# HamidGadirov/OpticalFlowSciVis

Measured on AMD Instinct MI355X. Metric: volume-pairs/sec, Flow-3D unsupervised train step (fwd+loss+bwd+AdamW), higher is better.
Workload: dtype f32

## Files before the change

include/flowsci_hip.h:

```cpp
#ifndef FLOWSCI_HIP_H
#define FLOWSCI_HIP_H

#ifdef __cplusplus
extern "C" {
#endif

typedef void* fs_stream_t;

enum {
  FS_OK = 0,
  FS_ERR_NULLPTR = 1,
  FS_ERR_SHAPE = 2,
  FS_ERR_ARG = 3,
  FS_ERR_LAUNCH = 4,
  FS_ERR_UNSUPPORTED = 5
};

#define FS_ABI_VERSION 330
int fs_version(void);
const char* fs_error_string(int code);

int fs_warp3d_fwd(const float* in, const float* flow, float* out,
                  int B, int C, const int* in_dhw, int D, int H, int W, fs_stream_t stream);
int fs_warp3d_bwd(const float* in, const float* flow, const float* grad_out,
// ... 188 lines not shown
long long fs_conv3d_fwd_dprelu_part_floats(int B, int Cout, int Do, int Ho, int Wo);
long long fs_conv3d_fwd_dprelu_part_floats_k3(int B, int Cout, int Do, int Ho, int Wo);
int fs_conv3d_fwd_dprelu(const float* x, const float* w, const float* act_y, const float* prelu_weight,
                         int num_prelu_weights, float* grad_act_y, float* grad_prelu_weight, float* grad_bias,
                         float* part, float* ws, int B, int Cin, int Cout, int Di, int Hi, int Wi, int Do, int Ho, int Wo,
                         int kernel, int stride, int pad, fs_stream_t stream);
int fs_conv3d_fwd_prelu(const float* x, const float* w, const float* bias, const float* prelu_weight,
                        const float* residual, float* y, float* z, float* ws,
                        int B, int Cin, int Cout, int Di, int Hi, int Wi, int Do, int Ho, int Wo,
                        int kernel, int stride, int pad, int num_prelu_weights, fs_stream_t stream);
int fs_conv3d_tr_prelu(const float* x, const float* w, const float* bias, const float* prelu_weight,
                       float* y, float* z, float* ws,
                       int B, int Cin, int Cout, int Di, int Hi, int Wi, int Dout, int Hout, int Wout,
                       int num_prelu_weights, fs_stream_t stream);
int fs_conv3d_tr_add(const float* x, const float* w, const float* bias, const float* addend, float* y,
                     float* ws, int B, int Cin, int Cout, int Di, int Hi, int Wi,
                     int Dout, int Hout, int Wout, fs_stream_t stream);
long long fs_conv3d_tr_ws_floats(int Cin, int Cout);
int fs_conv3d_tr(const float* x, const float* w, const float* bias, float* y, float* ws,
                 int B, int Cin, int Cout, int Di, int Hi, int Wi, int Dout, int Hout, int Wout,
                 fs_stream_t stream);

#define FS_PRELU_MAX_CHUNKS 64
int fs_prelu_bwd(const float* x, const float* grad_out, const float* weight,
                 float* grad_x, float* grad_weight, float* grad_bias, float* ws,
                 int B, int C, int S, int num_weights, fs_stream_t stream);

int fs_conv3d_wrw(const float* g, const float* src, float* dw, int B, int Cg, int Cs,
                  int Do, int Ho, int Wo, int Di, int Hi, int Wi,
                  int kernel, int stride, int pad, fs_stream_t stream);
enum { FS_WRW_KERNEL_BRICK = 0,
       FS_WRW_KERNEL_DMA = 1,
       FS_WRW_KERNEL_WINO23 = 2,
       FS_WRW_KERNEL_WINO43 = 3    };
int fs_conv3d_wrw_kernel_id(const float* g, const float* src, int B, int Cg, int Cs,
                            int Do, int Ho, int Wo, int Di, int Hi, int Wi, int kernel, int stride, int pad);

int fs_conv3d_fwd_prelu_ms(const float* const* src, const long long* batch_strides, const float* w, const float* bias,
                           const float* prelu_weight, float* y, float* z, float* ws,
                           int B, int Cin, int Cout, int Di, int Hi, int Wi, int Do, int Ho, int Wo,
                           int kernel, int stride, int pad, int num_prelu_weights, fs_stream_t stream);
int fs_conv3d_wrw_ms(const float* g, const float* const* src, const long long* batch_strides, float* dw,
                     int B, int Cg, int Cs, int Do, int Ho, int Wo, int Di, int Hi, int Wi,
                     int kernel, int stride, int pad, fs_stream_t stream);

long long fs_conv3d_wrw_det_ws_floats(const float* g, const float* src, const float* const* src_planes,
                                      const long long* batch_strides, int B, int Cg, int Cs,
                                      int Do, int Ho, int Wo, int Di, int Hi, int Wi, int kernel, int stride, int pad);
int fs_conv3d_wrw_det(const float* g, const float* src, const float* const* src_planes, const long long* batch_strides,
                      float* dw, float* ws, long long ws_floats, int B, int Cg, int Cs,
                      int Do, int Ho, int Wo, int Di, int Hi, int Wi, int kernel, int stride, int pad,
                      fs_stream_t stream);

typedef struct FsWprepJob {
  const float* w;
  float* ws;
  int kind;
  int total;
  int p[6];
} FsWprepJob;
int fs_conv3d_fwd_wprep_jobs(FsWprepJob* jobs_host, int cap, const float* x, const float* w, float* ws,
                             int B, int Cin, int Cout, int Di, int Hi, int Wi, int Do, int Ho, int Wo,
                             int kernel, int stride, int pad, int wmode);
int fs_conv3d_tr_wprep_jobs(FsWprepJob* jobs_host, int cap, const float* x, const float* w, float* ws, int B, int Cin,
                            int Cout, int Di, int Hi, int Wi, int Dout, int Hout, int Wout, int has_prelu_out);
int fs_conv3d_wprep_batch(const FsWprepJob* jobs_dev, int njobs, fs_stream_t stream);

// ... 5 lines not shown
```

opticalflowscivis_amd/csrc/convwrw.hip:

```cpp
#include <cstdint>
#include <cstdlib>
#include <type_traits>

#include "common.hpp"

namespace {

typedef float f32x16 __attribute__((ext_vector_type(16)));

constexpr int KW = 32;

struct WP {
  int B, Cg, Cs;
  int Do, Ho, Wo;
  int Di, Hi, Wi;
  int pad;
  int segs;
  long long steps;
  int spw;
  int nsrc = 0;
  const float* const* srcv = nullptr;
  const long long* sbsv = nullptr;
};

struct WB {
  int B, Cg, Cs;
  int Do, Ho, Wo, Di, Hi, Wi;
  int pad;
  int bz, by, bx;
  long long bricks;
  int spw;
  int nsrc;
  const float* src[12];
  long long sbs[12];
  long long slab;
};

struct WDet {
  float* ws;
  long long cap;
  long long* need;
};

__global__ __launch_bounds__(256) void wrw_reduce_kernel(const float* __restrict__ ws, int runs, long long n,
                                                         float* __restrict__ dW) {
  for (long long i = (long long)blockIdx.x * 256 + threadIdx.x; i < n; i += (long long)gridDim.x * 256) {
    float a = ws[i];
    for (int r = 1; r < runs; ++r) a += ws[(size_t)r * n + i];
    dW[i] = a;
  }
}

static inline int wrw_det_begin(const WDet* det, long long runs, long long dwf, float* dW, float** out, long long* p_slab) {
  *out = dW; *p_slab = 0;
  if (det == nullptr) return -1;
  if (det->need != nullptr) { *det->need = runs * dwf; return FS_OK; }
  if (det->ws == nullptr || runs * dwf > det->cap) return FS_ERR_ARG;
  *out = det->ws; *p_slab = dwf;
  return -1;
}

static inline void wrw_det_end(const WDet* det, long long runs, long long dwf, float* dW, hipStream_t st) {
  if (det == nullptr || det->need != nullptr) return;
  const long long blocks = (dwf + 255) / 256;
  hipLaunchKernelGGL(wrw_reduce_kernel, dim3((unsigned)(blocks < 4096 ? blocks : 4096)), dim3(256), 0, st, det->ws, (int)runs,
                     dwf, dW);
}

// ... 204 lines not shown
  if (want < 1) want = 1;
  long long spw = (p.bricks + want - 1) / want;
  if (spw < 2) spw = 2;
  p.spw = (int)(spw > (1 << 20) ? (1 << 20) : spw);
  const long long gx = (p.bricks + p.spw - 1) / p.spw;
  if (gx >= (1ll << 31) || nchunks > 65535 || mtiles > 65535) return FS_ERR_SHAPE;
  dim3 grid((unsigned)gx, nchunks, mtiles);
  constexpr int K3 = K * K * K;
  float* out;
  const long long dwf = (long long)p.Cg * p.Cs * K3;
  const int drc = wrw_det_begin(det, gx, dwf, dW, &out, &p.slab);
  if (drc >= 0) return drc;
  if (mt == 2)
    hipLaunchKernelGGL((conv3d_wrw_brick_kernel<K, S, NC, 2, TZ, TY>), grid, dim3(256), 0, st, G, Src, out, p);
  else
    hipLaunchKernelGGL((conv3d_wrw_brick_kernel<K, S, NC, 1, TZ, TY>), grid, dim3(256), 0, st, G, Src, out, p);
  wrw_det_end(det, gx, dwf, dW, st);
  FS_LAUNCH_CHECK();
  return FS_OK;
}


typedef __attribute__((address_space(3))) void* lds_ptr_t;
constexpr unsigned DMA_OOB = 0x80000000u;
#ifdef FS_WRW_STAMPS
__device__ unsigned long long fs_wrw_dbg[4 * 8];
#define STAMP(i) do { const unsigned long long now_ = __builtin_amdgcn_s_memtime(); dt[i] += now_ - tprev; tprev = now_; } while (0)
#else
#define STAMP(i) do { } while (0)
#endif

constexpr int up4(int n) { return (n + 3) / 4 * 4; }

template <int K, int S, int NC, int MT, int TZ, int TY, int FULL, int HALF, int KWX = 32>
__global__ __launch_bounds__(512, 2) void conv3d_wrw_dma_kernel(const float* __restrict__ G,
                                                             const float* __restrict__ Src,
                                                             float* __restrict__ dW, WB p) {
  constexpr int K3 = K * K * K;
  constexpr int NTOT = NC * K3;
  constexpr int NT32 = 4 * FULL + 2 * HALF;
  static_assert(NT32 * 32 >= NTOT && (NT32 - 1) * 32 < NTOT + 32, "column tiles cover the chunk");
  static_assert(HALF == 0 || MT == 2, "a shared column tile is split by row tile");
  constexpr int NB = FULL + HALF;
  constexpr int ROWS = TZ * TY;
  static_assert(KWX == 32 || KWX == 16, "brick x extent");
  constexpr int YR = KW / KWX;
  constexpr int TYB = TY * YR;
  constexpr int ZT = (TZ - 1) * S + K, YT = (TYB - 1) * S + K;
  constexpr int XL = 4;
  constexpr int XP = up4(XL + (KWX - 1) * S + K);
  constexpr int PSP = YT * XP, CHSP = ZT * PSP;
  constexpr int GP = ROWS * KW + 4;
  constexpr int NGF = 32 * MT * GP;
  constexpr int NGL = (NGF + 255) / 256 * 256;
  constexpr int NSF = NC * CHSP;
  constexpr int NSL = (NSF + 255) / 256 * 256;
  constexpr int NGW = (NGL / 256 + 3) / 4;
  constexpr int NSW = (NSL / 256 + 3) / 4;
  constexpr int BUF = NGL + NSL;
  static_assert(2 * BUF * 4 <= 160 * 1024, "two buffers fit the CU's LDS");
  __shared__ __attribute__((aligned(16))) float lds[2 * BUF];

  const int t = threadIdx.x, lane = t & 63;
  const int wave = __builtin_amdgcn_readfirstlane(t >> 6);
  const int wv = wave & 3;
  const bool loader = wave >= 4;
  const int l31 = lane & 31, kh = lane >> 5;
  const int c0 = blockIdx.y * NC;
  const int g0 = blockIdx.z * 32 * MT;
  const size_t gvol = (size_t)p.Do * p.Ho * p.Wo, svol = (size_t)p.Di * p.Hi * p.Wi;
  const long long s0 = (long long)blockIdx.x * p.spw;
  const long long s1 = min(s0 + p.spw, p.bricks);

  if (loader) {
#if defined(__HIP_DEVICE_COMPILE__)
    __builtin_amdgcn_s_setprio(3);
    unsigned soff[NSW], scls[NSW];
    int sch[NSW];
    const int zhi = p.Di + p.pad - (p.bz - 1) * TZ * S, yhi = p.Hi + p.pad - (p.by - 1) * TYB * S,
              xhi = p.Wi + XL - (p.bx - 1) * KWX * S;
#pragma unroll
    for (int k = 0; k < NSW; ++k) {
      const int q = 256 * (wv + 4 * k) + 4 * lane;
      const int c = q / CHSP, r1 = q - c * CHSP;
      const int z = r1 / PSP, r2 = r1 - z * PSP;
      const int y = r2 / XP, x = r2 - y * XP;
      const bool ok = q < NSF && c0 + c < p.Cs;
      soff[k] = ok ? ((p.nsrc ? 0u : (unsigned)c * (unsigned)svol) + ((unsigned)z * p.Hi + (unsigned)y) * p.Wi + (unsigned)x) * 4u
                   : DMA_OOB;
      sch[k] = q < NSF ? c : NC - 1;
      scls[k] = (z < p.pad ? 1u : 0u) | (z >= zhi ? 2u : 0u) | (y < p.pad ? 4u : 0u) | (y >= yhi ? 8u : 0u) |
                (x < XL ? 16u : 0u) | (x >= xhi ? 32u : 0u);
    }
    unsigned goff[NGW], gpk[NGW];
#pragma unroll
    for (int k = 0; k < NGW; ++k) {
      const int f = 256 * (wv + 4 * k) + 4 * lane;
      const int r = f / GP, w = f - r * GP;
      const int row = w / KW, e = w % KW;
      const int rz = row / TY, ry = (row % TY) * YR + e / KWX, col = e % KWX;
      const bool ok = f < NGF && w < ROWS * KW && g0 + r < p.Cg;
      goff[k] = ok ? ((unsigned)r * (unsigned)gvol + (unsigned)((rz * p.Ho + ry) * p.Wo + col)) * 4u : DMA_OOB;
      gpk[k] = (unsigned)rz | ((unsigned)ry << 8) | ((unsigned)col << 16);
    }
    const bool g_exact = p.Do % TZ == 0 && p.Ho % TYB == 0 && p.Wo % KWX == 0;
    int bxi, byi, bzi, b;
    {
// ... 38 lines not shown
        __amdgpu_buffer_rsrc_t rc[NC];
#pragma unroll
        for (int c = 0; c < NC; ++c) {
          const bool live = c0 + c < p.Cs;
          const int ch = live ? c0 + c : 0;
          rc[c] = __builtin_amdgcn_make_buffer_rsrc((void*)(p.src[ch] + (size_t)b * (size_t)p.sbs[ch] + org), (short)0,
                                                    live ? 0x7fffffff : 0, 0x00020000);
        }
#pragma unroll
        for (int k = 0; k < NSW; ++k) {
          if (256 * (wv + 4 * k) < NSL) {
            const unsigned vo = (scls[k] & bmask) == 0u ? soff[k] : DMA_OOB;
#pragma unroll
            for (int c = 0; c < NC; ++c)
              if (256 * (wv + 4 * k) < (c + 1) * CHSP && 256 * (wv + 4 * k) + 256 > c * CHSP)
                if (sch[k] == c)
                  __builtin_amdgcn_raw_ptr_buffer_load_lds(rc[c], (lds_ptr_t)(dbase + NGL + 256 * (wv + 4 * k)), 16, vo, 0, 0, 0);
          }
        }
      }
      if (++bxi == p.bx) { bxi = 0; if (++byi == p.by) { byi = 0; if (++bzi == p.bz) { bzi = 0; ++b; } } }
    };
    if (s0 < s1) stage(0);
    asm volatile("s_waitcnt vmcnt(0)" ::: "memory");
    __builtin_amdgcn_s_barrier();
    int buf = 0;
    for (long long st = s0; st < s1; ++st) {
      if (st + 1 < s1) stage(buf ^ 1);
      asm volatile("s_waitcnt vmcnt(0)" ::: "memory");
      __builtin_amdgcn_s_barrier();
      buf ^= 1;
    }
#else
    (void)gvol; (void)svol; (void)NGW; (void)NSW; (void)DMA_OOB;
#endif
    return;
  }

  int boff[NB];
#pragma unroll
  for (int n = 0; n < NB; ++n) {
    const int tile = (n < FULL) ? wv * FULL + n : 4 * FULL + (wv >> 1);
    const int j = tile * 32 + l31;
    int off = 0;
    if (j < NTOT) {
      const int c = j / K3, r = j - c * K3;
      const int kz = r / (K * K), ky = (r / K) % K, kx = r % K;
      off = c * CHSP + kz * PSP + ky * XP + kx;
    }
    boff[n] = off + XL - p.pad;
  }

  f32x16 acc[FULL > 0 ? FULL : 1][MT];
  f32x16 acch;
#pragma unroll
  for (int r = 0; r < 16; ++r) {
    acch[r] = 0.f;
#pragma unroll
    for (int n = 0; n < FULL; ++n)
#pragma unroll
      for (int m = 0; m < MT; ++m) acc[n][m][r] = 0.f;
  }

  __builtin_amdgcn_s_barrier();
  int buf = 0;
#ifdef FS_WRW_STAMPS
  unsigned long long dt[8] = {0, 0, 0, 0, 0, 0, 0, 0};
  unsigned long long tprev = __builtin_amdgcn_s_memtime();
// ... 65 lines not shown

template <int K, int S, int NC, int MT, int TZ, int TY, int FULL, int HALF, int KWX = 32>
int launch_dma(const float* G, const float* Src, float* dW, const WP& w, hipStream_t st, const WDet* det = nullptr) {
  WB p;
  p.B = w.B; p.Cg = w.Cg; p.Cs = w.Cs; p.Do = w.Do; p.Ho = w.Ho; p.Wo = w.Wo;
  p.Di = w.Di; p.Hi = w.Hi; p.Wi = w.Wi; p.pad = w.pad;
  p.nsrc = w.nsrc;
  for (int c = 0; c < w.nsrc; ++c) { p.src[c] = w.srcv[c]; p.sbs[c] = w.sbsv[c]; }
  p.bz = fs::cdiv(p.Do, TZ); p.by = fs::cdiv(p.Ho, TY * (KW / KWX)); p.bx = fs::cdiv(p.Wo, KWX);
  p.bricks = (long long)p.B * p.bz * p.by * p.bx;
  const int mtiles = fs::cdiv(p.Cg, 32 * MT);
  const int nchunks = fs::cdiv(p.Cs, NC);
  long long want = 256 / ((long long)mtiles * nchunks);
  if (want < 1) want = 1;
  long long spw = (p.bricks + want - 1) / want;
  if (spw < 1) spw = 1;
  p.spw = (int)(spw > (1 << 20) ? (1 << 20) : spw);
  const long long gx = (p.bricks + p.spw - 1) / p.spw;
  if (gx >= (1ll << 31) || nchunks > 65535 || mtiles > 65535) return FS_ERR_SHAPE;
  constexpr int K3 = K * K * K;
  float* out;
  const long long dwf = (long long)p.Cg * p.Cs * K3;
  const int drc = wrw_det_begin(det, gx, dwf, dW, &out, &p.slab);
  if (drc >= 0) return drc;
  hipLaunchKernelGGL((conv3d_wrw_dma_kernel<K, S, NC, MT, TZ, TY, FULL, HALF, KWX>), dim3((unsigned)gx, nchunks, mtiles),
                     dim3(512), 0, st, G, Src, out, p);
  wrw_det_end(det, gx, dwf, dW, st);
  FS_LAUNCH_CHECK();
  return FS_OK;
}

#include "convwrwwino.hpp"
#include "convwrwwino4.hpp"

}

#ifdef FS_WRW_STAMPS
extern "C" int fs_debug_wrw_stamps(unsigned long long* out) {
  return hipMemcpyFromSymbol(out, HIP_SYMBOL(fs_wrw_dbg), sizeof(unsigned long long) * 32) == hipSuccess ? 0 : 1;
}
#endif

#define FS_WRW_PICK(id, ...)        \
  do {                              \
    if (plan != nullptr) { *plan = (id); return FS_OK; } \
    return __VA_ARGS__;             \
  } while (0)

static int conv3d_wrw_impl(const float* g, const float* src, const float* const* srcv, const long long* sbsv, float* dw,
                           int B, int Cg, int Cs, int Do, int Ho, int Wo, int Di, int Hi, int Wi, int kernel, int stride,
                           int pad, fs_stream_t stream, int* plan = nullptr, const WDet* det = nullptr) {
  FS_REQUIRE_PTR(g);
  if (plan == nullptr) FS_REQUIRE_PTR(dw);
  if (srcv == nullptr) FS_REQUIRE_PTR(src);
  if (B < 1 || Cg < 1 || Cs < 1 || Do < 1 || Ho < 1 || Wo < 1 || Di < 1 || Hi < 1 || Wi < 1)
    return FS_ERR_SHAPE;
  if (!((kernel == 3 && stride == 1) || (kernel == 4 && stride == 2)) || pad < 0 || pad >= kernel)
    return FS_ERR_ARG;
  if ((Do - 1) * stride + kernel > Di + 2 * pad || (Ho - 1) * stride + kernel > Hi + 2 * pad ||
      (Wo - 1) * stride + kernel > Wi + 2 * pad)
    return FS_ERR_SHAPE;
  if ((long long)64 * Do * Ho * Wo * 4 >= (1ll << 32) || (long long)8 * Di * Hi * Wi * 4 >= (1ll << 32))
    return FS_ERR_SHAPE;
  WP p;
  p.B = B; p.Cg = Cg; p.Cs = Cs; p.Do = Do; p.Ho = Ho; p.Wo = Wo; p.Di = Di; p.Hi = Hi; p.Wi = Wi;
  p.pad = pad;
  p.segs = fs::cdiv(Wo, KW);
  p.steps = (long long)B * Do * Ho * p.segs;
  bool ms_aligned = true;
  if (srcv != nullptr) {
    if (Cs > 12) return FS_ERR_UNSUPPORTED;
    p.nsrc = Cs; p.srcv = srcv; p.sbsv = sbsv;
    for (int c = 0; c < Cs; ++c) {
      if (srcv[c] == nullptr) return FS_ERR_NULLPTR;
      if (sbsv[c] < (long long)Di * Hi * Wi) return FS_ERR_ARG;
      ms_aligned = ms_aligned && ((uintptr_t)srcv[c] & 15) == 0 && sbsv[c] % 4 == 0;
    }
  }
  hipStream_t st = (hipStream_t)stream;
  static const bool reg_only = FS_AB_ENV("FLOWSCI_WRW_REG");
  const bool dma_ok = !reg_only && pad <= stride && (Wo >= KW || Wo == 16) && Wo % 4 == 0 && Wi % 4 == 0 &&
                      (((uintptr_t)g | (srcv ? (uintptr_t)0 : (uintptr_t)src)) & 15) == 0 && ms_aligned &&
                      (long long)64 * Do * Ho * Wo * 4 < (1ll << 31) && (long long)16 * Di * Hi * Wi * 4 < (1ll << 31);
  if (srcv != nullptr) {
    if (dma_ok && kernel == 4 && Cg <= 32 && Cs >= 3 && Wo >= KW) FS_WRW_PICK(FS_WRW_KERNEL_DMA, launch_dma<4, 2, 6, 1, 2, 2, 3, 0>(g, src, dw, p, st, det));
    return FS_ERR_UNSUPPORTED;
  }
  if (dma_ok && wrw_wino4_ok(p, g, src, kernel, stride)) FS_WRW_PICK(FS_WRW_KERNEL_WINO43, launch_wrw_wino4(g, src, dw, p, st, det));
#ifdef FS_ABLATION
  if (dma_ok && det == nullptr && wrw_wino_ok(p, g, src, kernel, stride)) FS_WRW_PICK(FS_WRW_KERNEL_WINO23, launch_wrw_wino(g, src, dw, p, st));
#endif
  if (dma_ok) {
    if (kernel == 3 && Cg > 32 && Cs >= 8 && Wo == 16) FS_WRW_PICK(FS_WRW_KERNEL_DMA, launch_dma<3, 1, 16, 2, 1, 4, 3, 1, 16>(g, src, dw, p, st, det));
    if (kernel == 3 && Cg > 32 && Cs >= 8) FS_WRW_PICK(FS_WRW_KERNEL_DMA, launch_dma<3, 1, 16, 2, 1, 4, 3, 1>(g, src, dw, p, st, det));
    if (kernel == 4 && Cg > 32 && Cs >= 4 && Wo == 16) FS_WRW_PICK(FS_WRW_KERNEL_DMA, launch_dma<4, 2, 8, 2, 1, 2, 4, 0, 16>(g, src, dw, p, st, det));
    if (kernel == 4 && Cg > 32 && Cs >= 4 && Wo >= KW) FS_WRW_PICK(FS_WRW_KERNEL_DMA, launch_dma<4, 2, 8, 2, 1, 2, 4, 0>(g, src, dw, p, st, det));
    if (kernel == 4 && Cg <= 32 && Cs >= 3 && Wo >= KW) FS_WRW_PICK(FS_WRW_KERNEL_DMA, launch_dma<4, 2, 6, 1, 2, 2, 3, 0>(g, src, dw, p, st, det));
    if (kernel == 4 && Cg <= 32 && Wo >= KW) FS_WRW_PICK(FS_WRW_KERNEL_DMA, launch_dma<4, 2, 2, 1, 2, 2, 1, 0>(g, src, dw, p, st, det));
  }
  if (kernel == 3) FS_WRW_PICK(FS_WRW_KERNEL_BRICK, launch_brick<3, 1, 8, 1, 4>(g, src, dw, p, st, det));
  const int cost2 = (Cs + 1) / 2, cost4 = 2 * ((Cs + 3) / 4);
  if (cost2 < cost4) FS_WRW_PICK(FS_WRW_KERNEL_BRICK, launch_brick<4, 2, 2, 1, 2>(g, src, dw, p, st, det));
  FS_WRW_PICK(FS_WRW_KERNEL_BRICK, launch_brick<4, 2, 4, 1, 2>(g, src, dw, p, st, det));
}

extern "C" int fs_conv3d_wrw_kernel_id(const float* g, const float* src, int B, int Cg, int Cs, int Do, int Ho, int Wo,
                                       int Di, int Hi, int Wi, int kernel, int stride, int pad) {
  int id = -1;
  const int rc = conv3d_wrw_impl(g, src, nullptr, nullptr, nullptr, B, Cg, Cs, Do, Ho, Wo, Di, Hi, Wi, kernel, stride, pad,
                                 nullptr, &id);
  return rc == FS_OK ? id : -rc;
}

extern "C" int fs_conv3d_wrw(const float* g, const float* src, float* dw, int B, int Cg, int Cs, int Do,
                             int Ho, int Wo, int Di, int Hi, int Wi, int kernel, int stride, int pad,
                             fs_stream_t stream) {
  FS_ENTER();
  return conv3d_wrw_impl(g, src, nullptr, nullptr, dw, B, Cg, Cs, Do, Ho, Wo, Di, Hi, Wi, kernel, stride, pad, stream);
}

extern "C" long long fs_conv3d_wrw_det_ws_floats(const float* g, const float* src, const float* const* src_planes,
                                                 const long long* batch_strides, int B, int Cg, int Cs, int Do, int Ho,
                                                 int Wo, int Di, int Hi, int Wi, int kernel, int stride, int pad) {
  long long need = 0;
  WDet det = {nullptr, 0, &need};
  float dummy;
  const int rc = conv3d_wrw_impl(g, src, src_planes, batch_strides, &dummy, B, Cg, Cs, Do, Ho, Wo, Di, Hi, Wi, kernel, stride,
// ... 24 lines not shown
```

opticalflowscivis_amd/ops.py:

```python
import ctypes

import torch

from . import _lib

WARP2D_RIFE, WARP2D_PWC, WARP2D_PHOTO, WARP2D_DILATED = 0, 1, 2, 3


def _stream(t):
    return torch.cuda.current_stream(t.device).cuda_stream


def _need_cuda_f32(name, t, ndim):
    if not isinstance(t, torch.Tensor):
        raise ValueError("%s must be a tensor" % name)
    if t.dtype != torch.float32:
        raise ValueError("%s must be float32, got %s" % (name, t.dtype))
    if t.dim() != ndim:
        raise ValueError("%s must be %d-D, got shape %s" % (name, ndim, tuple(t.shape)))
    if not t.is_cuda:
        raise ValueError("%s must live on a GPU (the HIP hot path has no CPU fallback); got %s" %
                         (name, t.device))
    return t.contiguous()

# ... 1499 lines not shown
    return 4 * _vol(in_dhw) * 4 < (1 << 32) and 8 * _vol(in_dhw) < (1 << 31)


def conv3d_wrw_fits(src_dhw, g_dhw):
    return 8 * _vol(src_dhw) * 4 < (1 << 32) and 64 * _vol(g_dhw) * 4 < (1 << 32)


_dw_arena = {}
_dw_need = {}


def _dw_zeros(like, shape):
    n = 1
    for v in shape:
        n *= int(v)
    if _prep_depth == 0 or not _PREP_ON or torch.cuda.is_current_stream_capturing():
        return like.new_zeros(shape)
    dev = like.device
    st = _dw_arena.get(dev)
    if st is None or st[0] != _prep_epoch:
        if st is not None:
            _dw_need[dev] = st[3]
        need = _dw_need.get(dev, 0)
        st = _dw_arena[dev] = [_prep_epoch, like.new_zeros(need) if need else None, 0, 0]
    pad = (n + 3) // 4 * 4
    st[3] += pad
    if st[1] is None or st[2] + pad > st[1].numel():
        return like.new_zeros(shape)
    out = st[1].narrow(0, st[2], n).view(shape)
    st[2] += pad
    return out


def _conv3d_wrw_det(g, src_ptr, pv, sv, geo, nbytes, flops, equiv, allow_unsupported=False):
    L = _lib.lib()
    need = int(L.fs_conv3d_wrw_det_ws_floats(g.data_ptr(), src_ptr, pv, sv, *geo))
    if need == -FS_ERR_UNSUPPORTED and allow_unsupported:
        return None
    if need < 0:
        _lib.check(-need, "fs_conv3d_wrw_det_ws_floats")
    B, Cg, Cs = geo[:3]
    k = geo[9]
    dw = g.new_empty(Cg, Cs, k, k, k)
    ws = g.new_empty(max(need, 1))
    with torch.cuda.device(g.device):
        _call("fs_conv3d_wrw_det", g.data_ptr(), src_ptr, pv, sv, dw.data_ptr(), ws.data_ptr(), need, *geo, _stream(g),
              algo_bytes=nbytes, algo_flops=flops, equiv_flops=equiv, record_as="fs_conv3d_wrw")
    return dw


def conv3d_wrw(g, src, k, stride, pad):
    g = _need_cuda_f32("g", g, 5)
    src = _need_cuda_f32("src", src, 5)
    B, Cg = g.shape[:2]
    Cs = src.shape[1]
    if src.shape[0] != B:
        raise ValueError("batch mismatch")
    fq = 2 * g.numel() * Cs * int(k) ** 3
    kid = conv3d_wrw_kernel_id(g.data_ptr(), src.data_ptr(), B, Cg, Cs, g.shape[2:], src.shape[2:], k, stride, pad)
    geo = (B, Cg, Cs, g.shape[2], g.shape[3], g.shape[4], src.shape[2], src.shape[3], src.shape[4], int(k), int(stride), int(pad))
    if torch.are_deterministic_algorithms_enabled():
        return _conv3d_wrw_det(g, src.data_ptr(), None, None, geo, 4 * (g.numel() + src.numel()),
                               {WRW_KERNEL_WINO43: fq // 2, WRW_KERNEL_WINO23: fq * 2 // 3}.get(kid, fq), fq)
    dw = _dw_zeros(g, (Cg, Cs, k, k, k))
    with torch.cuda.device(g.device):
        _call("fs_conv3d_wrw", g.data_ptr(), src.data_ptr(), dw.data_ptr(), B, Cg, Cs, g.shape[2],
              g.shape[3], g.shape[4], src.shape[2], src.shape[3], src.shape[4], int(k), int(stride),
              int(pad), _stream(g), algo_bytes=4 * (g.numel() + src.numel()),
              algo_flops={WRW_KERNEL_WINO43: fq // 2, WRW_KERNEL_WINO23: fq * 2 // 3}.get(kid, fq), equiv_flops=fq,
              kernel="conv3d_wrw_wino4_kernel<0>" if kid == WRW_KERNEL_WINO43 else None)
    return dw


WRW_KERNEL_BRICK, WRW_KERNEL_DMA, WRW_KERNEL_WINO23, WRW_KERNEL_WINO43 = 0, 1, 2, 3


def conv3d_wrw_kernel_id(g_ptr, src_ptr, B, Cg, Cs, g_dhw, src_dhw, k, stride, pad):
    kid = int(_lib.lib().fs_conv3d_wrw_kernel_id(int(g_ptr), int(src_ptr), int(B), int(Cg), int(Cs),
                                                 *(int(v) for v in g_dhw), *(int(v) for v in src_dhw), int(k), int(stride),
                                                 int(pad)))
    if kid < 0:
        _lib.check(-kid, "fs_conv3d_wrw_kernel_id")
    return kid


def conv3d_wrw_takes_winograd(B, Cg, Cs, g_dhw, src_dhw, k, stride, pad, g_misalign=0, src_misalign=0):
    return conv3d_wrw_kernel_id(0x1000 + g_misalign, 0x1000 + src_misalign, B, Cg, Cs, g_dhw, src_dhw, k, stride,
                                pad) in (WRW_KERNEL_WINO23, WRW_KERNEL_WINO43)


FS_ERR_UNSUPPORTED = 5


def _channel_planes(pieces):
    B, dhw = pieces[0].shape[0], tuple(pieces[0].shape[2:])
    vol = dhw[0] * dhw[1] * dhw[2]
    inner = (vol, dhw[1] * dhw[2], dhw[2], 1)
    ptrs, strides = [], []
    for t in pieces:
        if (not isinstance(t, torch.Tensor) or not t.is_cuda or t.dtype != torch.float32 or t.dim() != 5 or
                t.shape[0] != B or tuple(t.shape[2:]) != dhw or tuple(t.stride()[1:]) != inner or
                t.stride(0) < t.shape[1] * vol or t.stride(0) % 4 or t.data_ptr() % 16 or vol % 4):
            return None
        for c in range(t.shape[1]):
            ptrs.append(t.data_ptr() + 4 * c * vol)
            strides.append(t.stride(0))
    n = len(ptrs)
# ... 13 lines not shown
    if w.shape[1] != Cin or tuple(w.shape[2:]) != (k, k, k):
        raise ValueError("weight %s does not fit %d input channels" % (tuple(w.shape), Cin))
    if bias is not None:
        bias = _need_cuda_f32("bias", bias, 1)
    x0 = pieces[0]
    B = x0.shape[0]
    Di, Hi, Wi = x0.shape[2:]
    Do, Ho, Wo = [(n + 2 * pad - k) // stride + 1 for n in (Di, Hi, Wi)]
    if min(Do, Ho, Wo) < 1:
        return None
    y = x0.new_empty((B, Cout, Do, Ho, Wo))
    z = torch.empty_like(y)
    wp, ws = _prepared_fwd(w, x0.data_ptr(), B, Cin, Cout, (Di, Hi, Wi), (Do, Ho, Wo), k, stride, pad, 0)
    xbytes = 4 * B * Cin * Di * Hi * Wi
    with torch.cuda.device(x0.device):
        rc = _call_rc("fs_conv3d_fwd_prelu_ms", pv, sv, wp, _ptr(bias), a.data_ptr(), y.data_ptr(), z.data_ptr(),
                   ws.data_ptr(), B, Cin, Cout, Di, Hi, Wi, Do, Ho, Wo, int(k), int(stride), int(pad), int(a.numel()),
                      _stream(x0), algo_bytes=xbytes + 8 * y.numel(), algo_flops=2 * y.numel() * Cin * int(k) ** 3,
                      record_as="fs_conv3d_fwd", allow=(FS_ERR_UNSUPPORTED,))
    if rc == FS_ERR_UNSUPPORTED:
        _prep_not_written()
        return None
    return y, z


def conv3d_wrw_ms(g, pieces, k, stride, pad):
    planes = _channel_planes(pieces)
    if planes is None:
        return None
    pv, sv, Cs = planes
    g = _need_cuda_f32("g", g, 5)
    B, Cg = g.shape[:2]
    Di, Hi, Wi = pieces[0].shape[2:]
    if torch.are_deterministic_algorithms_enabled():
        geo = (B, Cg, Cs, g.shape[2], g.shape[3], g.shape[4], Di, Hi, Wi, int(k), int(stride), int(pad))
        fq = 2 * g.numel() * Cs * int(k) ** 3
        return _conv3d_wrw_det(g, 0, pv, sv, geo, 4 * (g.numel() + B * Cs * Di * Hi * Wi), fq, fq, allow_unsupported=True)
    dw = _dw_zeros(g, (Cg, Cs, k, k, k))
    with torch.cuda.device(g.device):
        rc = _call_rc("fs_conv3d_wrw_ms", g.data_ptr(), pv, sv, dw.data_ptr(), B, Cg, Cs, g.shape[2], g.shape[3], g.shape[4],
                   Di, Hi, Wi, int(k), int(stride), int(pad), _stream(g),
                      algo_bytes=4 * (g.numel() + B * Cs * Di * Hi * Wi), algo_flops=2 * g.numel() * Cs * int(k) ** 3,
                      record_as="fs_conv3d_wrw", allow=(FS_ERR_UNSUPPORTED,))
    if rc == FS_ERR_UNSUPPORTED:
        return None
    return dw


def conv3d_deconv_grad_input_dprelu(gy, w, act_y, prelu_weight):
    gy = _need_cuda_f32("grad_output", gy, 5)
    w = _need_cuda_f32("w", w, 5)
    act_y = _need_cuda_f32("act_y", act_y, 5)
    a = _need_cuda_f32("prelu_weight", prelu_weight, 1)
    B, Cg = gy.shape[:2]
    Cin_t = w.shape[0]
    if w.shape[1] != Cg or tuple(w.shape[2:]) != (4, 4, 4) or act_y.shape[1] != Cin_t or a.numel() not in (1, Cin_t):
        raise ValueError("shapes do not describe a k4 s2 deconvolution: gy %s w %s act_y %s" %
                         (tuple(gy.shape), tuple(w.shape), tuple(act_y.shape)))
    Di, Hi, Wi = gy.shape[2:]
    Do, Ho, Wo = act_y.shape[2:]
    if any((n + 2 - 4) // 2 + 1 != m for n, m in zip((Di, Hi, Wi), (Do, Ho, Wo))) or Cin_t > 32:
        return None
    L = _lib.lib()
    npart = int(L.fs_conv3d_fwd_dprelu_part_floats(B, Cin_t, Do, Ho, Wo))
    if npart < 0:
        return None
    out = torch.empty_like(act_y)
    ga, gb = torch.empty_like(a), act_y.new_empty(Cin_t)
    part = act_y.new_empty(npart)
    wp, ws = _prepared_fwd(w, gy.data_ptr(), B, Cg, Cin_t, (Di, Hi, Wi), (Do, Ho, Wo), 4, 2, 1, 0)
    nb = 4 * (gy.numel() + 2 * out.numel())
    fl = 2 * out.numel() * Cg * 64
    with torch.cuda.device(gy.device):
        args = (gy.data_ptr(), wp, act_y.data_ptr(), a.data_ptr(), a.numel(), out.data_ptr(), ga.data_ptr(),
                gb.data_ptr(), part.data_ptr(), ws.data_ptr(), B, Cg, Cin_t, Di, Hi, Wi, Do, Ho, Wo, 4, 2, 1, _stream(gy))
# ... 226 lines not shown
```

Before: 27.93.

## Add split-bf16x3 MFMA weight-gradient kernel for stride-2 k4 convolutions

Adds a new weight-gradient kernel for 4x4x4 stride-2 3D convolutions. It splits each fp32 operand into three bf16 pieces and accumulates six bf16 MFMA products, approximating fp32 accuracy on the matrix cores instead of the existing fp32 path. The DMA loader is factored into a shared device function so both kernels reuse the LDS double-buffered pipeline. The new kernel is selected by default ahead of the old DMA kernel and can be disabled through an environment variable. It adds extra split arithmetic per operand and slightly reduced precision compared with pure fp32.

```diff
diff --git a/include/flowsci_hip.h b/include/flowsci_hip.h
--- a/include/flowsci_hip.h
+++ b/include/flowsci_hip.h
@@ -244,7 +244,8 @@
 enum { FS_WRW_KERNEL_BRICK = 0,
        FS_WRW_KERNEL_DMA = 1,
        FS_WRW_KERNEL_WINO23 = 2,
-       FS_WRW_KERNEL_WINO43 = 3    };
+       FS_WRW_KERNEL_WINO43 = 3,
+       FS_WRW_KERNEL_S3 = 4        };
 int fs_conv3d_wrw_kernel_id(const float* g, const float* src, int B, int Cg, int Cs,
                             int Do, int Ho, int Wo, int Di, int Hi, int Wi, int kernel, int stride, int pad);
 
diff --git a/opticalflowscivis_amd/csrc/convwrw.hip b/opticalflowscivis_amd/csrc/convwrw.hip
--- a/opticalflowscivis_amd/csrc/convwrw.hip
+++ b/opticalflowscivis_amd/csrc/convwrw.hip
@@ -34,6 +34,7 @@
   const float* src[12];
   long long sbs[12];
   long long slab;
+  int ab;
 };
 
 struct WDet {
@@ -304,47 +305,38 @@
 
 constexpr int up4(int n) { return (n + 3) / 4 * 4; }
 
-template <int K, int S, int NC, int MT, int TZ, int TY, int FULL, int HALF, int KWX = 32>
-__global__ __launch_bounds__(512, 2) void conv3d_wrw_dma_kernel(const float* __restrict__ G,
-                                                             const float* __restrict__ Src,
-                                                             float* __restrict__ dW, WB p) {
-  constexpr int K3 = K * K * K;
-  constexpr int NTOT = NC * K3;
-  constexpr int NT32 = 4 * FULL + 2 * HALF;
-  static_assert(NT32 * 32 >= NTOT && (NT32 - 1) * 32 < NTOT + 32, "column tiles cover the chunk");
-  static_assert(HALF == 0 || MT == 2, "a shared column tile is split by row tile");
-  constexpr int NB = FULL + HALF;
-  constexpr int ROWS = TZ * TY;
+template <int K, int S, int NC, int MT, int TZ, int TY, int KWX>
+struct WrwDmaGeom {
   static_assert(KWX == 32 || KWX == 16, "brick x extent");
-  constexpr int YR = KW / KWX;
-  constexpr int TYB = TY * YR;
-  constexpr int ZT = (TZ - 1) * S + K, YT = (TYB - 1) * S + K;
-  constexpr int XL = 4;
-  constexpr int XP = up4(XL + (KWX - 1) * S + K);
-  constexpr int PSP = YT * XP, CHSP = ZT * PSP;
-  constexpr int GP = ROWS * KW + 4;
-  constexpr int NGF = 32 * MT * GP;
-  constexpr int NGL = (NGF + 255) / 256 * 256;
-  constexpr int NSF = NC * CHSP;
-  constexpr int NSL = (NSF + 255) / 256 * 256;
-  constexpr int NGW = (NGL / 256 + 3) / 4;
-  constexpr int NSW = (NSL / 256 + 3) / 4;
-  constexpr int BUF = NGL + NSL;
+  static constexpr int ROWS = TZ * TY;
+  static constexpr int YR = KW / KWX;
+  static constexpr int TYB = TY * YR;
+  static constexpr int ZT = (TZ - 1) * S + K, YT = (TYB - 1) * S + K;
+  static constexpr int XL = 4;
+  static constexpr int XP = up4(XL + (KWX - 1) * S + K);
+  static constexpr int PSP = YT * XP, CHSP = ZT * PSP;
+  static constexpr int GP = ROWS * KW + 4;
+  static constexpr int NGF = 32 * MT * GP;
+  static constexpr int NGL = (NGF + 255) / 256 * 256;
+  static constexpr int NSF = NC * CHSP;
+  static constexpr int NSL = (NSF + 255) / 256 * 256;
+  static constexpr int NGW = (NGL / 256 + 3) / 4;
+  static constexpr int NSW = (NSL / 256 + 3) / 4;
+  static constexpr int BUF = NGL + NSL;
   static_assert(2 * BUF * 4 <= 160 * 1024, "two buffers fit the CU's LDS");
-  __shared__ __attribute__((aligned(16))) float lds[2 * BUF];
-
-  const int t = threadIdx.x, lane = t & 63;
-  const int wave = __builtin_amdgcn_readfirstlane(t >> 6);
-  const int wv = wave & 3;
-  const bool loader = wave >= 4;
-  const int l31 = lane & 31, kh = lane >> 5;
+};
+
+template <int K, int S, int NC, int MT, int TZ, int TY, int KWX>
+__device__ __forceinline__ void wrw_dma_loader(const float* __restrict__ G, const float* __restrict__ Src, const WB& p,
+                                               float* lds, int wv, int lane, long long s0, long long s1) {
+  using Geo = WrwDmaGeom<K, S, NC, MT, TZ, TY, KWX>;
+  constexpr int ROWS = Geo::ROWS, YR = Geo::YR, TYB = Geo::TYB, XL = Geo::XL, XP = Geo::XP, PSP = Geo::PSP,
+                CHSP = Geo::CHSP, GP = Geo::GP, NGF = Geo::NGF, NGL = Geo::NGL, NSF = Geo::NSF, NSL = Geo::NSL,
+                NGW = Geo::NGW, NSW = Geo::NSW, BUF = Geo::BUF;
   const int c0 = blockIdx.y * NC;
   const int g0 = blockIdx.z * 32 * MT;
   const size_t gvol = (size_t)p.Do * p.Ho * p.Wo, svol = (size_t)p.Di * p.Hi * p.Wi;
-  const long long s0 = (long long)blockIdx.x * p.spw;
-  const long long s1 = min(s0 + p.spw, p.bricks);
-
-  if (loader) {
+  {
 #if defined(__HIP_DEVICE_COMPILE__)
     __builtin_amdgcn_s_setprio(3);
     unsigned soff[NSW], scls[NSW];
@@ -449,8 +441,40 @@
       buf ^= 1;
     }
 #else
-    (void)gvol; (void)svol; (void)NGW; (void)NSW; (void)DMA_OOB;
+    (void)G; (void)Src; (void)p; (void)lds; (void)wv; (void)lane; (void)s0; (void)s1; (void)c0; (void)g0; (void)gvol; (void)svol;
+    (void)ROWS; (void)YR; (void)TYB; (void)XL; (void)XP; (void)PSP; (void)CHSP; (void)GP; (void)NGF; (void)NGL; (void)NSF;
+    (void)NSL; (void)NGW; (void)NSW; (void)BUF; (void)DMA_OOB;
 #endif
+  }
+}
+
+template <int K, int S, int NC, int MT, int TZ, int TY, int FULL, int HALF, int KWX = 32>
+__global__ __launch_bounds__(512, 2) void conv3d_wrw_dma_kernel(const float* __restrict__ G,
+                                                             const float* __restrict__ Src,
+                                                             float* __restrict__ dW, WB p) {
+  constexpr int K3 = K * K * K;
+  constexpr int NTOT = NC * K3;
+  constexpr int NT32 = 4 * FULL + 2 * HALF;
+  static_assert(NT32 * 32 >= NTOT && (NT32 - 1) * 32 < NTOT + 32, "column tiles cover the chunk");
+  static_assert(HALF == 0 || MT == 2, "a shared column tile is split by row tile");
+  constexpr int NB = FULL + HALF;
+  using Geo = WrwDmaGeom<K, S, NC, MT, TZ, TY, KWX>;
+  constexpr int ROWS = Geo::ROWS, YR = Geo::YR, XL = Geo::XL, XP = Geo::XP, PSP = Geo::PSP, CHSP = Geo::CHSP,
+                GP = Geo::GP, NGL = Geo::NGL, BUF = Geo::BUF;
+  __shared__ __attribute__((aligned(16))) float lds[2 * BUF];
+
+  const int t = threadIdx.x, lane = t & 63;
+  const int wave = __builtin_amdgcn_readfirstlane(t >> 6);
+  const int wv = wave & 3;
+  const bool loader = wave >= 4;
+  const int l31 = lane & 31, kh = lane >> 5;
+  const int c0 = blockIdx.y * NC;
+  const int g0 = blockIdx.z * 32 * MT;
+  const long long s0 = (long long)blockIdx.x * p.spw;
+  const long long s1 = min(s0 + p.spw, p.bricks);
+
+  if (loader) {
+    wrw_dma_loader<K, S, NC, MT, TZ, TY, KWX>(G, Src, p, lds, wv, lane, s0, s1);
     return;
   }
 
@@ -582,6 +606,7 @@
 
 #include "convwrwwino.hpp"
 #include "convwrwwino4.hpp"
+#include "convwrw_s3.hpp"
 
 }
 
@@ -632,8 +657,12 @@
   const bool dma_ok = !reg_only && pad <= stride && (Wo >= KW || Wo == 16) && Wo % 4 == 0 && Wi % 4 == 0 &&
                       (((uintptr_t)g | (srcv ? (uintptr_t)0 : (uintptr_t)src)) & 15) == 0 && ms_aligned &&
                       (long long)64 * Do * Ho * Wo * 4 < (1ll << 31) && (long long)16 * Di * Hi * Wi * 4 < (1ll << 31);
+  static const bool no_s3 = FS_AB_ENV("FLOWSCI_WRW_NO_S3");
   if (srcv != nullptr) {
-    if (dma_ok && kernel == 4 && Cg <= 32 && Cs >= 3 && Wo >= KW) FS_WRW_PICK(FS_WRW_KERNEL_DMA, launch_dma<4, 2, 6, 1, 2, 2, 3, 0>(g, src, dw, p, st, det));
+    if (dma_ok && kernel == 4 && Cg <= 32 && Cs >= 3 && Wo >= KW) {
+      if (!no_s3) FS_WRW_PICK(FS_WRW_KERNEL_S3, launch_wrw_s3<6, 1, 2, 2, 3, 0>(g, src, dw, p, st, det));
+      FS_WRW_PICK(FS_WRW_KERNEL_DMA, launch_dma<4, 2, 6, 1, 2, 2, 3, 0>(g, src, dw, p, st, det));
+    }
     return FS_ERR_UNSUPPORTED;
   }
   if (dma_ok && wrw_wino4_ok(p, g, src, kernel, stride)) FS_WRW_PICK(FS_WRW_KERNEL_WINO43, launch_wrw_wino4(g, src, dw, p, st, det));
@@ -643,6 +672,11 @@
   if (dma_ok) {
     if (kernel == 3 && Cg > 32 && Cs >= 8 && Wo == 16) FS_WRW_PICK(FS_WRW_KERNEL_DMA, launch_dma<3, 1, 16, 2, 1, 4, 3, 1, 16>(g, src, dw, p, st, det));
     if (kernel == 3 && Cg > 32 && Cs >= 8) FS_WRW_PICK(FS_WRW_KERNEL_DMA, launch_dma<3, 1, 16, 2, 1, 4, 3, 1>(g, src, dw, p, st, det));
+    if (!no_s3) {
+      if (kernel == 4 && Cg > 32 && Cs >= 4 && Wo == 16) FS_WRW_PICK(FS_WRW_KERNEL_S3, launch_wrw_s3<8, 2, 1, 2, 4, 0, 16>(g, src, dw, p, st, det));
+      if (kernel == 4 && Cg > 32 && Cs >= 4 && Wo >= KW) FS_WRW_PICK(FS_WRW_KERNEL_S3, launch_wrw_s3<8, 2, 1, 2, 4, 0>(g, src, dw, p, st, det));
+      if (kernel == 4 && Cg <= 32 && Cs >= 3 && Wo >= KW) FS_WRW_PICK(FS_WRW_KERNEL_S3, launch_wrw_s3<6, 1, 2, 2, 3, 0>(g, src, dw, p, st, det));
+    }
     if (kernel == 4 && Cg > 32 && Cs >= 4 && Wo == 16) FS_WRW_PICK(FS_WRW_KERNEL_DMA, launch_dma<4, 2, 8, 2, 1, 2, 4, 0, 16>(g, src, dw, p, st, det));
     if (kernel == 4 && Cg > 32 && Cs >= 4 && Wo >= KW) FS_WRW_PICK(FS_WRW_KERNEL_DMA, launch_dma<4, 2, 8, 2, 1, 2, 4, 0>(g, src, dw, p, st, det));
     if (kernel == 4 && Cg <= 32 && Cs >= 3 && Wo >= KW) FS_WRW_PICK(FS_WRW_KERNEL_DMA, launch_dma<4, 2, 6, 1, 2, 2, 3, 0>(g, src, dw, p, st, det));
diff --git a/opticalflowscivis_amd/csrc/convwrw_s3.hpp b/opticalflowscivis_amd/csrc/convwrw_s3.hpp
--- /dev/null
+++ b/opticalflowscivis_amd/csrc/convwrw_s3.hpp
@@ -0,0 +1,243 @@
+#pragma once
+
+typedef __bf16 w3_bf16x8 __attribute__((ext_vector_type(8)));
+typedef unsigned w3_u32x4 __attribute__((ext_vector_type(4)));
+typedef float w3_f32x4 __attribute__((ext_vector_type(4)));
+
+__device__ __forceinline__ unsigned w3_pack(float a, float b) {
+  typedef __bf16 bf16x2_t __attribute__((ext_vector_type(2)));
+  const bf16x2_t h = {(__bf16)a, (__bf16)b};
+  return __builtin_bit_cast(unsigned, h);
+}
+
+__device__ __forceinline__ void w3_split(const float (&v)[8], w3_bf16x8 (&h)[3], int ab) {
+  unsigned w[3][4];
+#pragma unroll
+  for (int i = 0; i < 4; ++i) {
+    float ra = v[2 * i], rc = v[2 * i + 1];
+#ifdef FS_ABLATION
+    if (ab & 1) {
+      w[0][i] = __float_as_uint(ra); w[1][i] = __float_as_uint(rc); w[2][i] = __float_as_uint(ra);
+      continue;
+    }
+#endif
+    w[0][i] = w3_pack(ra, rc);
+    ra -= __uint_as_float(w[0][i] << 16); rc -= __uint_as_float(w[0][i] & 0xffff0000u);
+    asm volatile("" : "+v"(ra), "+v"(rc));
+    w[1][i] = w3_pack(ra, rc);
+    ra -= __uint_as_float(w[1][i] << 16); rc -= __uint_as_float(w[1][i] & 0xffff0000u);
+    asm volatile("" : "+v"(ra), "+v"(rc));
+    w[2][i] = w3_pack(ra, rc);
+  }
+  (void)ab;
+#pragma unroll
+  for (int pc = 0; pc < 3; ++pc) {
+    const w3_u32x4 u = {w[pc][0], w[pc][1], w[pc][2], w[pc][3]};
+    h[pc] = __builtin_bit_cast(w3_bf16x8, u);
+  }
+}
+
+template <int NC, int MT, int TZ, int TY, int FULL, int HALF, int KWX = 32>
+__global__ __launch_bounds__(512, 2) void conv3d_wrw_s3_kernel(const float* __restrict__ G,
+                                                            const float* __restrict__ Src,
+                                                            float* __restrict__ dW, WB p) {
+  constexpr int K = 4, S = 2;
+  constexpr int K3 = K * K * K;
+  constexpr int NTOT = NC * K3;
+  constexpr int NT32 = 4 * FULL + 2 * HALF;
+  static_assert(NT32 * 32 >= NTOT && (NT32 - 1) * 32 < NTOT + 32, "column tiles cover the chunk");
+  static_assert(HALF == 0 || MT == 2, "a shared column tile is split by row tile");
+  constexpr int NB = FULL + HALF;
+  using Geo = WrwDmaGeom<K, S, NC, MT, TZ, TY, KWX>;
+  constexpr int ROWS = Geo::ROWS, YR = Geo::YR, XL = Geo::XL, XP = Geo::XP, PSP = Geo::PSP, CHSP = Geo::CHSP,
+                GP = Geo::GP, NGL = Geo::NGL, BUF = Geo::BUF;
+  __shared__ __attribute__((aligned(16))) float lds[2 * BUF];
+
+  const int t = threadIdx.x, lane = t & 63;
+  const int wave = __builtin_amdgcn_readfirstlane(t >> 6);
+  const int wv = wave & 3;
+  const int l31 = lane & 31, kh = lane >> 5;
+  const int c0 = blockIdx.y * NC;
+  const int g0 = blockIdx.z * 32 * MT;
+  const long long s0 = (long long)blockIdx.x * p.spw;
+  const long long s1 = min(s0 + p.spw, p.bricks);
+
+  if (wave >= 4) {
+    wrw_dma_loader<K, S, NC, MT, TZ, TY, KWX>(G, Src, p, lds, wv, lane, s0, s1);
+    return;
+  }
+
+  int boff[NB];
+#pragma unroll
+  for (int n = 0; n < NB; ++n) {
+    const int tile = (n < FULL) ? wv * FULL + n : 4 * FULL + (wv >> 1);
+    const int j = tile * 32 + l31;
+    int off = 0;
+    if (j < NTOT) {
+      const int c = j / K3, r = j - c * K3;
+      const int kz = r / (K * K), ky = (r / K) % K, kx = r % K;
+      off = c * CHSP + kz * PSP + ky * XP + kx;
+    }
+    boff[n] = off + XL - p.pad + 8 * kh * S;
+  }
+  const int aoff = l31 * GP + 8 * kh;
+  const int hoff = ((wv & 1) * 32 + l31) * GP + 8 * kh;
+  const int ab = p.ab;
+
+  f32x16 acc[FULL > 0 ? FULL : 1][MT];
+  f32x16 acch;
+#pragma unroll
+  for (int r = 0; r < 16; ++r) {
+    acch[r] = 0.f;
+#pragma unroll
+    for (int n = 0; n < FULL; ++n)
+#pragma unroll
+      for (int m = 0; m < MT; ++m) acc[n][m][r] = 0.f;
+  }
+
+  __builtin_amdgcn_s_barrier();
+  int buf = 0;
+  for (long long st = s0; st < s1; ++st) {
+    const float* sG = lds + buf * BUF;
+    const float* sS = sG + NGL;
+    constexpr int NQ = ROWS * (KW / 16), NU = NQ * NB;
+    auto srow = [&](int q) {
+      const int row = q >> 1, hq = q & 1;
+      return (row / TY) * S * PSP + ((row % TY) * YR + (KWX == 16 ? hq : 0)) * S * XP + (KWX == 32 ? 16 * hq * S : 0);
+    };
+    auto read_a = [&](int q, float (&ra)[MT][8], float (&rh)[8]) {
+      const int gb = (q >> 1) * KW + 16 * (q & 1);
+#pragma unroll
+      for (int m = 0; m < MT; ++m) {
+        const w3_f32x4 lo = *reinterpret_cast<const w3_f32x4*>(sG + m * 32 * GP + aoff + gb);
+        const w3_f32x4 hi = *reinterpret_cast<const w3_f32x4*>(sG + m * 32 * GP + aoff + gb + 4);
+#pragma unroll
+        for (int i = 0; i < 4; ++i) { ra[m][i] = lo[i]; ra[m][4 + i] = hi[i]; }
+      }
+      if (HALF) {
+        const w3_f32x4 lo = *reinterpret_cast<const w3_f32x4*>(sG + hoff + gb);
+        const w3_f32x4 hi = *reinterpret_cast<const w3_f32x4*>(sG + hoff + gb + 4);
+#pragma unroll
+        for (int i = 0; i < 4; ++i) { rh[i] = lo[i]; rh[4 + i] = hi[i]; }
+      }
+    };
+    auto read_b = [&](int u, float (&rb)[8]) {
+      const float* q = sS + boff[u % NB] + srow(u / NB);
+#pragma unroll
+      for (int i = 0; i < 8; ++i) rb[i] = q[S * i];
+    };
+    constexpr int PA[6] = {2, 0, 1, 1, 0, 0}, PB[6] = {0, 2, 1, 0, 1, 0};
+    w3_bf16x8 pa[2][MT][3], ph[2][3], pb[2][3];
+    float ra[MT][8], rh[8], rb[8];
+    read_a(0, ra, rh);
+    read_b(0, rb);
+#pragma unroll
+    for (int m = 0; m < MT; ++m) w3_split(ra[m], pa[0][m], ab);
+    if (HALF) w3_split(rh, ph[0], ab);
+    w3_split(rb, pb[0], ab);
+    if (NU > 1) {
+      if (NB == 1) read_a(1, ra, rh);
+      read_b(1, rb);
+    }
+#pragma unroll
+    for (int u = 0; u < NU; ++u) {
+      __builtin_amdgcn_sched_barrier(0);
+      const int q = u / NB, n = u % NB;
+#ifdef FS_ABLATION
+      if (!(ab & 2))
+#endif
+      {
+        if (n < FULL) {
+#pragma unroll
+          for (int q6 = 0; q6 < 6; ++q6)
+#pragma unroll
+            for (int m = 0; m < MT; ++m)
+              acc[n][m] = __builtin_amdgcn_mfma_f32_32x32x16_bf16(pa[q & 1][m][PA[q6]], pb[u & 1][PB[q6]], acc[n][m], 0, 0, 0);
+        } else {
+#pragma unroll
+          for (int q6 = 0; q6 < 6; ++q6) acch = __builtin_amdgcn_mfma_f32_32x32x16_bf16(ph[q & 1][PA[q6]], pb[u & 1][PB[q6]], acch, 0, 0, 0);
+        }
+      }
+      if (u + 1 < NU) {
+        if ((u + 1) % NB == 0) {
+#pragma unroll
+          for (int m = 0; m < MT; ++m) w3_split(ra[m], pa[(q + 1) & 1][m], ab);
+          if (HALF) w3_split(rh, ph[(q + 1) & 1], ab);
+        }
+        w3_split(rb, pb[(u + 1) & 1], ab);
+      }
+      if (u + 2 < NU) {
+        if ((u + 2) % NB == 0) read_a((u + 2) / NB, ra, rh);
+        read_b(u + 2, rb);
+      }
+#ifdef FS_ABLATION
+      if (ab & 2) {
+#pragma unroll
+        for (int pc = 0; pc < 3; ++pc) {
+          asm volatile("" ::"v"(pb[u & 1][pc]));
+#pragma unroll
+          for (int m = 0; m < MT; ++m) asm volatile("" ::"v"(pa[q & 1][m][pc]));
+          if (HALF) asm volatile("" ::"v"(ph[q & 1][pc]));
+        }
+      }
+#endif
+    }
+    __builtin_amdgcn_s_barrier();
+    buf ^= 1;
+  }
+
+  auto flush = [&](const f32x16& a, int tile, int m) {
+    const int j = tile * 32 + l31;
+    if (j >= NTOT || c0 * K3 + j >= p.Cs * K3) return;
+#pragma unroll
+    for (int r = 0; r < 16; ++r) {
+      const int g = g0 + m * 32 + (r & 3) + 8 * (r >> 2) + 4 * kh;
+      if (g < p.Cg) {
+        float* q = dW + (size_t)blockIdx.x * p.slab + (size_t)g * p.Cs * K3 + (size_t)c0 * K3 + j;
+        if (p.slab) *q = a[r]; else atomicAdd(q, a[r]);
+      }
+    }
+  };
+#pragma unroll
+  for (int n = 0; n < FULL; ++n)
+#pragma unroll
+    for (int m = 0; m < MT; ++m) flush(acc[n][m], wv * FULL + n, m);
+  if (HALF) flush(acch, 4 * FULL + (wv >> 1), wv & 1);
+}
+
+template <int NC, int MT, int TZ, int TY, int FULL, int HALF, int KWX = 32>
+int launch_wrw_s3(const float* G, const float* Src, float* dW, const WP& w, hipStream_t st, const WDet* det = nullptr) {
+  constexpr int K = 4;
+  WB p;
+  p.B = w.B; p.Cg = w.Cg; p.Cs = w.Cs; p.Do = w.Do; p.Ho = w.Ho; p.Wo = w.Wo;
+  p.Di = w.Di; p.Hi = w.Hi; p.Wi = w.Wi; p.pad = w.pad;
+  p.nsrc = w.nsrc;
+  for (int c = 0; c < w.nsrc; ++c) { p.src[c] = w.srcv[c]; p.sbs[c] = w.sbsv[c]; }
+  p.bz = fs::cdiv(p.Do, TZ); p.by = fs::cdiv(p.Ho, TY * (KW / KWX)); p.bx = fs::cdiv(p.Wo, KWX);
+  p.bricks = (long long)p.B * p.bz * p.by * p.bx;
+  const int mtiles = fs::cdiv(p.Cg, 32 * MT);
+  const int nchunks = fs::cdiv(p.Cs, NC);
+  long long want = 256 / ((long long)mtiles * nchunks);
+  if (want < 1) want = 1;
+  long long spw = (p.bricks + want - 1) / want;
+  if (spw < 1) spw = 1;
+  p.spw = (int)(spw > (1 << 20) ? (1 << 20) : spw);
+  const long long gx = (p.bricks + p.spw - 1) / p.spw;
+  if (gx >= (1ll << 31) || nchunks > 65535 || mtiles > 65535) return FS_ERR_SHAPE;
+#ifdef FS_ABLATION
+  static const int s3_ab = (int)FS_AB_ENV_LL("FLOWSCI_WRW_S3_AB", 0);
+  p.ab = s3_ab;
+#else
+  p.ab = 0;
+#endif
+  constexpr int K3 = K * K * K;
+  float* out;
+  const long long dwf = (long long)p.Cg * p.Cs * K3;
+  const int drc = wrw_det_begin(det, gx, dwf, dW, &out, &p.slab);
+  if (drc >= 0) return drc;
+  hipLaunchKernelGGL((conv3d_wrw_s3_kernel<NC, MT, TZ, TY, FULL, HALF, KWX>), dim3((unsigned)gx, nchunks, mtiles), dim3(512), 0,
+                     st, G, Src, out, p);
+  wrw_det_end(det, gx, dwf, dW, st);
+  FS_LAUNCH_CHECK();
+  return FS_OK;
+}
diff --git a/opticalflowscivis_amd/ops.py b/opticalflowscivis_amd/ops.py
--- a/opticalflowscivis_amd/ops.py
+++ b/opticalflowscivis_amd/ops.py
@@ -1555,7 +1555,7 @@
     return out
 
 
-def _conv3d_wrw_det(g, src_ptr, pv, sv, geo, nbytes, flops, equiv, allow_unsupported=False):
+def _conv3d_wrw_det(g, src_ptr, pv, sv, geo, nbytes, flops, equiv, allow_unsupported=False, kernel=None):
     L = _lib.lib()
     need = int(L.fs_conv3d_wrw_det_ws_floats(g.data_ptr(), src_ptr, pv, sv, *geo))
     if need == -FS_ERR_UNSUPPORTED and allow_unsupported:
@@ -1568,7 +1568,7 @@
     ws = g.new_empty(max(need, 1))
     with torch.cuda.device(g.device):
         _call("fs_conv3d_wrw_det", g.data_ptr(), src_ptr, pv, sv, dw.data_ptr(), ws.data_ptr(), need, *geo, _stream(g),
-              algo_bytes=nbytes, algo_flops=flops, equiv_flops=equiv, record_as="fs_conv3d_wrw")
+              algo_bytes=nbytes, algo_flops=flops, equiv_flops=equiv, record_as="fs_conv3d_wrw", kernel=kernel)
     return dw
 
 
@@ -1582,20 +1582,29 @@
     fq = 2 * g.numel() * Cs * int(k) ** 3
     kid = conv3d_wrw_kernel_id(g.data_ptr(), src.data_ptr(), B, Cg, Cs, g.shape[2:], src.shape[2:], k, stride, pad)
     geo = (B, Cg, Cs, g.shape[2], g.shape[3], g.shape[4], src.shape[2], src.shape[3], src.shape[4], int(k), int(stride), int(pad))
+    fl = {WRW_KERNEL_WINO43: fq // 2, WRW_KERNEL_WINO23: fq * 2 // 3, WRW_KERNEL_S3: 6 * fq}.get(kid, fq)
     if torch.are_deterministic_algorithms_enabled():
-        return _conv3d_wrw_det(g, src.data_ptr(), None, None, geo, 4 * (g.numel() + src.numel()),
-                               {WRW_KERNEL_WINO43: fq // 2, WRW_KERNEL_WINO23: fq * 2 // 3}.get(kid, fq), fq)
+        return _conv3d_wrw_det(g, src.data_ptr(), None, None, geo, 4 * (g.numel() + src.numel()), fl, fq,
+                               kernel=_wrw_s3_symbol(kid, Cg, g.shape[4]))
     dw = _dw_zeros(g, (Cg, Cs, k, k, k))
     with torch.cuda.device(g.device):
         _call("fs_conv3d_wrw", g.data_ptr(), src.data_ptr(), dw.data_ptr(), B, Cg, Cs, g.shape[2],
               g.shape[3], g.shape[4], src.shape[2], src.shape[3], src.shape[4], int(k), int(stride),
               int(pad), _stream(g), algo_bytes=4 * (g.numel() + src.numel()),
-              algo_flops={WRW_KERNEL_WINO43: fq // 2, WRW_KERNEL_WINO23: fq * 2 // 3}.get(kid, fq), equiv_flops=fq,
-              kernel="conv3d_wrw_wino4_kernel<0>" if kid == WRW_KERNEL_WINO43 else None)
+              algo_flops=fl, equiv_flops=fq,
+              kernel="conv3d_wrw_wino4_kernel<0>" if kid == WRW_KERNEL_WINO43 else _wrw_s3_symbol(kid, Cg, g.shape[4]))
     return dw
 
 
-WRW_KERNEL_BRICK, WRW_KERNEL_DMA, WRW_KERNEL_WINO23, WRW_KERNEL_WINO43 = 0, 1, 2, 3
+def _wrw_s3_symbol(kid, Cg, Wo):
+    if kid != WRW_KERNEL_S3:
+        return None
+    if int(Cg) > 32:
+        return "conv3d_wrw_s3_kernel<8, 2, 1, 2, 4, 0, %d>" % (16 if int(Wo) == 16 else 32)
+    return "conv3d_wrw_s3_kernel<6, 1, 2, 2, 3, 0, 32>"
+
+
+WRW_KERNEL_BRICK, WRW_KERNEL_DMA, WRW_KERNEL_WINO23, WRW_KERNEL_WINO43, WRW_KERNEL_S3 = 0, 1, 2, 3, 4
 
 
 def conv3d_wrw_kernel_id(g_ptr, src_ptr, B, Cg, Cs, g_dhw, src_dhw, k, stride, pad):
@@ -1675,15 +1684,19 @@
     g = _need_cuda_f32("g", g, 5)
     B, Cg = g.shape[:2]
     Di, Hi, Wi = pieces[0].shape[2:]
+    fq = 2 * g.numel() * Cs * int(k) ** 3
+    kid = conv3d_wrw_kernel_id(g.data_ptr(), pieces[0].data_ptr(), B, Cg, Cs, g.shape[2:], (Di, Hi, Wi), k, stride, pad)
+    sym = _wrw_s3_symbol(kid, Cg, g.shape[4])
+    fl = 6 * fq if sym is not None else fq
     if torch.are_deterministic_algorithms_enabled():
         geo = (B, Cg, Cs, g.shape[2], g.shape[3], g.shape[4], Di, Hi, Wi, int(k), int(stride), int(pad))
-        fq = 2 * g.numel() * Cs * int(k) ** 3
-        return _conv3d_wrw_det(g, 0, pv, sv, geo, 4 * (g.numel() + B * Cs * Di * Hi * Wi), fq, fq, allow_unsupported=True)
+        return _conv3d_wrw_det(g, 0, pv, sv, geo, 4 * (g.numel() + B * Cs * Di * Hi * Wi), fl, fq, allow_unsupported=True,
+                               kernel=sym)
     dw = _dw_zeros(g, (Cg, Cs, k, k, k))
     with torch.cuda.device(g.device):
         rc = _call_rc("fs_conv3d_wrw_ms", g.data_ptr(), pv, sv, dw.data_ptr(), B, Cg, Cs, g.shape[2], g.shape[3], g.shape[4],
                    Di, Hi, Wi, int(k), int(stride), int(pad), _stream(g),
-                      algo_bytes=4 * (g.numel() + B * Cs * Di * Hi * Wi), algo_flops=2 * g.numel() * Cs * int(k) ** 3,
+                      algo_bytes=4 * (g.numel() + B * Cs * Di * Hi * Wi), algo_flops=fl, equiv_flops=fq, kernel=sym,
                       record_as="fs_conv3d_wrw", allow=(FS_ERR_UNSUPPORTED,))
     if rc == FS_ERR_UNSUPPORTED:
         return None
```

After: 29.58 (median of 6 runs). +5.9%, better.
